# HarryL-Git/ampnet

Measured on AMD Instinct MI355X. Metric: AMPConv edges/sec (fwd+bwd), higher is better.
Workload: dtype f32

## Files before the change

### ampnet_amd/csrc/edge_mfma_bf16.hip

```cpp
#include "edge_wave16.h"

namespace {
using namespace wave16;

typedef unsigned short bf16_t;


#define MFMA_BF16(a, b, c) \
  __builtin_amdgcn_mfma_f32_16x16x32_bf16(__builtin_bit_cast(bf16x8, a), __builtin_bit_cast(bf16x8, b), (c), 0, 0, 0)

struct Args {
  ampconv_view_t Q, K, V, dO, O, dK, dV;
  const int32_t *ptr, *idx, *qidx;
  const float *cinv;
  HubArgs hub;
  int64_t n_units;
  int L, H;
  float qscale, oscale;
};

template <bool HALF>
__device__ __forceinline__ void store_tile(const ampconv_view_t &v, int64_t node, int h, const f32x4 (&T)[2][2],
                                           float scale, bool to_f32, int L, int lane) {
  const int g = lane >> 4;
#pragma unroll
  for (int nt = 0; nt < 2; ++nt) {
    const int i = (lane & 15) + 16 * nt;
    if (i < L) {
#pragma unroll
      for (int mc = 0; mc < (HALF ? 1 : 2); ++mc) {
        const float a = T[mc][nt][0] * scale, b = T[mc][nt][1] * scale, c = T[mc][nt][2] * scale,
                    d = T[mc][nt][3] * scale;
        const int64_t off = node * v.node_stride + (int64_t)h * v.head_stride + (int64_t)i * v.row_stride +
                            4 * g + 16 * mc;
        if (to_f32)
          *reinterpret_cast<float4 *>(reinterpret_cast<float *>(v.ptr) + off) = make_float4(a, b, c, d);
        else
          *reinterpret_cast<i32x2 *>(reinterpret_cast<bf16_t *>(v.ptr) + off) =
              i32x2{cvt_pk_bf16(a, b), cvt_pk_bf16(c, d)};
      }
    }
  }
}

struct FmtB {
  using Args = ::Args;
  static constexpr int kPlanes = 1, kElemBytes = 2, kLoOff = 0, kTileBytes = kPlaneBytes;
  using Frag = wave16::Frag<1>;
  template <bool HALF> using Geom = PairGeom<4, 3, HALF ? 2 : 4, 1>;
  static constexpr bool kHalfZeroLds = false;
  template <bool HALF> static constexpr int mc_tiles() { return 2; }
  static constexpr bool kShadow = false;
  static constexpr float kMasked = kNegBig, kPMul = 1.f;

  static __device__ __forceinline__ f32x4 mma(const Frag &a, const Frag &b, f32x4 c) { return MFMA_BF16(a.p[0], b.p[0], c); }
  static __device__ __forceinline__ Frag cd_frag(const f32x4 &t0, const f32x4 &t1) {
    return Frag{{i32x4{cvt_pk_bf16(t0[0], t0[1]), cvt_pk_bf16(t0[2], t0[3]), cvt_pk_bf16(t1[0], t1[1]),
                       cvt_pk_bf16(t1[2], t1[3])}}};
  }

  struct Scales {
    float sc;
  };
  template <bool HALF> static __device__ __forceinline__ Scales scales(const Args &a) { return Scales{a.qscale}; }
  static __device__ __forceinline__ int64_t qrow(const Args &a, int64_t r) { return a.qidx ? uniform_ld(a.qidx + r) : r; }
  static __device__ __forceinline__ float fwd_scale(const Scales &, float mean) { return mean; }
  static __device__ __forceinline__ float ds_mul(const Args &, int deg, const Frag (&)[2]) {
    return deg > 0 ? 1.f / (float)deg : 0.f;
  }
  template <bool HALF> static __device__ __forceinline__ float dq_scale(const Args &a, const Scales &, float, bool hubp) {
    return hubp ? 1.f : a.oscale;
  }

  template <bool HALF>
  static __device__ __forceinline__ float store(const ampconv_view_t &v, int64_t node, int h, const f32x4 (&T)[2][2],
                                                float scale, bool hubp, int L, int lane) {
    store_tile<HALF>(v, node, h, T, scale, hubp, L, lane);
    return 0.f;
  }
  template <bool HALF>
  static __device__ __forceinline__ void store_zero(const ampconv_view_t &v, int64_t node, int h, int L, int lane) {
    f32x4 Z[2][2];
#pragma unroll
    for (int mc = 0; mc < 2; ++mc) Z[mc][0] = Z[mc][1] = f32x4{0.f, 0.f, 0.f, 0.f};
    store_tile<HALF>(v, node, h, Z, 0.f, false, L, lane);
  }
  static __device__ __forceinline__ void record_absmax(const Args &, float) {}
};

template <bool FULL, bool HALF>
__global__ __launch_bounds__(64 * kWavesPerBlock) void fwd_bf16(Args a) { fwd_body<FmtB, FULL, HALF>(a); }
template <bool FULL, bool HALF>
__global__ __launch_bounds__(64 * kWavesPerBlock) void bwd_dst_bf16(Args a) { bwd_dst_body<FmtB, FULL, false, HALF>(a); }

constexpr int kTile32 = 32 * kRowBytes;

__device__ __forceinline__ i32x4 rowfrag_plain(const char *tile, int nt, int lane) {
  const int n = lane & 15, kg = lane >> 4;
  return *reinterpret_cast<const i32x4 *>(tile + plane_off(16 * nt + n, kg));
}
__device__ __forceinline__ i32x4 colfrag32(const char *tile, int blk, int lane) {
  const int q = (lane >> 2) & 3, pp = lane & 3, kg = lane >> 4;
  const int ch = 2 * blk + (pp >> 1), half = (pp & 1) << 3;
  return tr_frag(tile + plane_off(8 * kg + q, ch) + half, tile + plane_off(8 * kg + 4 + q, ch) + half);
}
__device__ __forceinline__ void file_column(char *img, int i, const f32x4 &t0, float t1_0, int g) {
  *reinterpret_cast<i32x2 *>(img + plane_off(i, g >> 1) + 8 * (g & 1)) = i32x2{cvt_pk_bf16(t0[0], t0[1]), cvt_pk_bf16(t0[2], t0[3])};
  *reinterpret_cast<unsigned short *>(img + plane_off(i, 2) + 2 * g) = (unsigned short)cvt_pk_bf16(t1_0, 0.f);
}

template <bool FULL, bool HALF>
__global__ __launch_bounds__(64 * kWavesPerBlock) void bwd_src_bf16_tr(Args a) {
  using G = FmtB::Geom<HALF>;
  __shared__ __attribute__((aligned(16))) char lds_all[kWavesPerBlock][4 * kTile32];
  for_unit<FmtB, HALF>(a, a.dK, &a.dV, [&](const Unit &u) __attribute__((always_inline)) {
    const int lane = u.lane, h = u.h, beg = u.beg, end = u.end;
    const int L = a.L, n = lane & 15, g = lane >> 4;
    char *Qt = lds_all[u.wave], *Gt = Qt + kTile32, *Pi = Gt + kTile32, *Si = Pi + kTile32;

    i32x4 kA[2], vA[2];
    {
      const char *kb = slot_ptr<2>(a.K, u.row, h), *vb = slot_ptr<2>(a.V, u.row, h);
      const unsigned krb = (unsigned)a.K.row_stride * 2u, vrb = (unsigned)a.V.row_stride * 2u;
#pragma unroll
      for (int mt = 0; mt < 2; ++mt) {
        kA[mt] = frag_global<1, HALF, true>(kb, krb, mt, L, lane).p[0];
        vA[mt] = frag_global<1, HALF, true>(vb, vrb, mt, L, lane).p[0];
      }
    }
    lds_zero(Qt, 4 * kTile32, lane);
    f32x4 dKT[2][2], dVT[2][2];
#pragma unroll
    for (int mc = 0; mc < 2; ++mc)
      dKT[mc][0] = dKT[mc][1] = dVT[mc][0] = dVT[mc][1] = f32x4{0.f, 0.f, 0.f, 0.f};

    Pair16<G::NLD> qg;
    float inv = 0.f, inv_next = 0.f;
    IdxWindow win;
    const unsigned qrb = (unsigned)a.Q.row_stride * 2u, grb = (unsigned)a.dO.row_stride * 2u;
    auto fetch = [&](int p, float &w) {
      const int64_t d = idxwin_get<true>(win, a.idx, a.cinv, p, end, lane, &w);
      pair16_load<FULL, G>(qg, slot_ptr<2>(a.Q, d, h), qrb, slot_ptr<2>(a.dO, d, h), grb, L, lane);
    };
    if (beg < end) {
      idxwin_load<true>(win, a.idx, a.cinv, beg, end, lane);
      fetch(beg, inv_next);
    }
    for (int p = beg; p < end; ++p) {
      pair16_to_lds<FULL, G, kTile32>(Qt, qg, L, lane);
      inv = inv_next;
      if (p + 1 < end) fetch(p + 1, inv_next);
      __builtin_amdgcn_wave_barrier();

      f32x4 S[2][2], dP[2][2];
#pragma unroll
      for (int nt = 0; nt < 2; ++nt) {
        const i32x4 qB = rowfrag_plain(Qt, nt, lane), gB = rowfrag_plain(Gt, nt, lane);
#pragma unroll
        for (int mt = 0; mt < 2; ++mt) {
          S[mt][nt] = MFMA_BF16(kA[mt], qB, (f32x4{0.f, 0.f, 0.f, 0.f}));
          dP[mt][nt] = MFMA_BF16(vA[mt], gB, (f32x4{0.f, 0.f, 0.f, 0.f}));
        }
      }
#pragma unroll
      for (int nt = 0; nt < 2; ++nt) {
        column_softmax<FULL>(S[0][nt], S[1][nt], a.qscale, 1.f, kNegBig, L, g);
        float part = S[1][nt][0] * dP[1][nt][0];
#pragma unroll
        for (int q = 0; q < 4; ++q) part = fmaf(S[0][nt][q], dP[0][nt][q], part);
        const float delta = groups_sum(part);
#pragma unroll
        for (int q = 0; q < 4; ++q) {
          dP[0][nt][q] = S[0][nt][q] * (dP[0][nt][q] - delta) * inv;
          S[0][nt][q] *= inv;
        }
        dP[1][nt][0] = S[1][nt][0] * (dP[1][nt][0] - delta) * inv;
        S[1][nt][0] *= inv;
        const int i = 16 * nt + n;
        if (i < kLmax && (FULL || i < L)) {
          file_column(Pi, i, S[0][nt], S[1][nt][0], g);
          file_column(Si, i, dP[0][nt], dP[1][nt][0], g);
        }
      }
      __builtin_amdgcn_wave_barrier();
      i32x4 pB[2], sB[2], gC[2], qC[2];
#pragma unroll
      for (int nt = 0; nt < 2; ++nt) {
        pB[nt] = colfrag32(Pi, nt, lane);
        sB[nt] = colfrag32(Si, nt, lane);
      }
#pragma unroll
      for (int mc = 0; mc < (HALF ? 1 : 2); ++mc) {
        gC[mc] = colfrag32(Gt, mc, lane);
        qC[mc] = colfrag32(Qt, mc, lane);
      }
      TR_FRAG_FENCE();
#pragma unroll
      for (int mc = 0; mc < (HALF ? 1 : 2); ++mc) {
        dVT[mc][0] = MFMA_BF16(gC[mc], pB[0], dVT[mc][0]);
        dVT[mc][1] = MFMA_BF16(gC[mc], pB[1], dVT[mc][1]);
        dKT[mc][0] = MFMA_BF16(qC[mc], sB[0], dKT[mc][0]);
        dKT[mc][1] = MFMA_BF16(qC[mc], sB[1], dKT[mc][1]);
      }
      __builtin_amdgcn_sched_barrier(0);
      asm volatile("s_nop 7" ::: "memory");
      __builtin_amdgcn_wave_barrier();
    }
    const bool hubp = a.hub.mode == 2;
    store_tile<HALF>(a.dK, u.onode, h, dKT, hubp ? 1.f : a.oscale, hubp, L, lane);
    store_tile<HALF>(a.dV, u.onode, h, dVT, 1.f, hubp, L, lane);
  });
}

typedef void (*EdgeKernel)(Args);
int launch(Args &a, int L, int D, int H, EdgeKernel const (&kernels)[2][2], hipStream_t stream) {
  const int dh = D / H;
  if (dh != DH && dh != DH / 2) return AMPCONV_E_BADARG;
  a.qscale = kLog2e / sqrtf((float)dh);
  a.oscale = 1.f / sqrtf((float)dh);
  return launch_wave16(kernels, a, L, dh == DH / 2, stream);
}

inline bool aligned16h(const ampconv_view_t &v) {
  return ((uintptr_t)v.ptr % 16 == 0) && (v.node_stride % 8 == 0) && (v.row_stride % 8 == 0) &&
         (v.head_stride % 8 == 0);
}

}

bool ampconv_bf16_supported(int L, int D, int H, const ampconv_view_t *views, int n) {
  if (!(L >= 1 && L <= kLmax && (D / H == DH || D / H == DH / 2) && D % H == 0)) return false;
  for (int i = 0; i < n; ++i)
    if (!aligned16h(views[i])) return false;
  return true;
}

int ampconv_fwd_edge_bf16(ampconv_view_t Q, ampconv_view_t K, ampconv_view_t V, const int32_t *rowptr,
                          const int32_t *col, const int32_t *qidx, int64_t n_rows, int L, int D, int H,
                          ampconv_view_t O, HubArgs hub, hipStream_t stream) {
  Args a{};
  a.Q = Q; a.K = K; a.V = V; a.O = O;
  a.ptr = rowptr; a.idx = col; a.qidx = qidx; a.hub = hub;
  a.n_units = n_rows * H; a.L = L; a.H = H;
  static const EdgeKernel kernels[2][2] = WAVE16_KERNELS(fwd_bf16);
  return launch(a, L, D, H, kernels, stream);
}

int ampconv_bwd_edge_dst_bf16(ampconv_view_t Q, ampconv_view_t K, ampconv_view_t V, ampconv_view_t dO,
                              const int32_t *rowptr, const int32_t *col, int64_t n_rows, int L, int D,
                              int H, ampconv_view_t dQ, HubArgs hub, hipStream_t stream) {
  Args a{};
  a.Q = Q; a.K = K; a.V = V; a.dO = dO; a.O = dQ;
  a.ptr = rowptr; a.idx = col; a.hub = hub;
  a.n_units = n_rows * H; a.L = L; a.H = H;
  static const EdgeKernel kernels[2][2] = WAVE16_KERNELS(bwd_dst_bf16);
  return launch(a, L, D, H, kernels, stream);
}

int ampconv_bwd_edge_src_bf16(ampconv_view_t Q, ampconv_view_t K, ampconv_view_t V, ampconv_view_t dO,
                              const int32_t *cscptr, const int32_t *crow, const float *cinv,
                              int64_t n_src, int L, int D, int H, ampconv_view_t dK, ampconv_view_t dV,
                              HubArgs hub, hipStream_t stream) {
  Args a{};
  a.Q = Q; a.K = K; a.V = V; a.dO = dO; a.dK = dK; a.dV = dV;
  a.ptr = cscptr; a.idx = crow; a.cinv = cinv; a.hub = hub;
  a.n_units = n_src * H; a.L = L; a.H = H;
  static const EdgeKernel kernels[2][2] = WAVE16_KERNELS(bwd_src_bf16_tr);
  return launch(a, L, D, H, kernels, stream);
}
```

### ampnet_amd/csrc/edge_mfma_f16x2.hip

```cpp
#include "edge_wave16.h"

namespace {
using namespace wave16;

constexpr int kLoOff = kPlaneBytes + 64;
constexpr int kTileBytes = kLoOff + kPlaneBytes;
constexpr float kPScale = 16384.f;
constexpr float kPUnscale = 1.f / 16384.f;
constexpr float kSqrtDh = 5.656854249492381f;
constexpr float kMasked = -__builtin_inff();

#define MFMA_F16(a, b, c) \
  __builtin_amdgcn_mfma_f32_16x16x32_f16(__builtin_bit_cast(f16x8, a), __builtin_bit_cast(f16x8, b), (c), 0, 0, 0)

__device__ __forceinline__ f32x4 mfma3(const i32x4 &ah, const i32x4 &al, const i32x4 &bh, const i32x4 &bl, f32x4 c) {
  c = MFMA_F16(al, bh, c);
  c = MFMA_F16(ah, bl, c);
  return MFMA_F16(ah, bh, c);
}

__device__ __forceinline__ float tile_max_norm2(const i32x4 &f0, const i32x4 &f1) {
  const float t = fmaxf(groups_sum(frag_sumsq(f0)), groups_sum(frag_sumsq(f1)));
  return __builtin_bit_cast(float, __builtin_amdgcn_readfirstlane(__builtin_bit_cast(int, row16_max(t))));
}
__device__ __forceinline__ float ds_scale(float own2, float other) {
  return plane_scale(2.f * __builtin_sqrtf(own2) * (kSqrtDh * other));
}

__device__ __forceinline__ void cd_frag2(const f32x4 &t0, float t1_0, i32x4 &hi, i32x4 &lo) {
  int h0, l0, h1, l1, h2, l2;
  split2(t0[0], t0[1], h0, l0);
  split2(t0[2], t0[3], h1, l1);
  split2(t1_0, 0.f, h2, l2);
  hi = i32x4{h0, h1, h2, 0};
  lo = i32x4{l0, l1, l2, 0};
}

struct Args {
  ampconv_view_t Q, K, V, dO, O, dK, dV;
  const int32_t *ptr, *idx;
  const float *bounds;
  float *absmax;
  const int32_t *spos;
  float *stats;
  HubArgs hub;
  int64_t n_units;
  int L, H;
};

template <bool QUARTER, int MC>
__device__ __forceinline__ float store_tile(const ampconv_view_t &v, int64_t node, int h, const f32x4 (&T)[MC][2],
                                            float scale, int L, int lane) {
  const int g = lane >> 4, n = lane & 15;
  float m = 0.f;
#pragma unroll
  for (int nt = 0; nt < 2; ++nt) {
    const int i = nt == 0 ? n : (QUARTER ? 16 + (n >> 2) : 16 + n);
    if (i < L && (nt == 0 || !QUARTER || (n & 3) == 0)) {
#pragma unroll
      for (int mc = 0; mc < MC; ++mc) {
        const float4 o = make_float4(T[mc][nt][0] * scale, T[mc][nt][1] * scale, T[mc][nt][2] * scale,
                                     T[mc][nt][3] * scale);
        const int64_t off = node * v.node_stride + (int64_t)h * v.head_stride + (int64_t)i * v.row_stride + 4 * g + 16 * mc;
        *reinterpret_cast<float4 *>(reinterpret_cast<float *>(v.ptr) + off) = o;
        m = finite_abs_max(m, o);
      }
    }
  }
  return m;
}

struct FmtP {
  using Args = ::Args;
  static constexpr int kPlanes = 2, kElemBytes = 4, kLoOff = ::kLoOff, kTileBytes = ::kTileBytes;
  using Frag = wave16::Frag<2>;
  template <bool HALF> using Geom = PairGeom<HALF ? 4 : 8, HALF ? 3 : 5, HALF ? 4 : 8, 2, ::kLoOff>;
  static constexpr bool kHalfZeroLds = true;
  template <bool HALF> static constexpr int mc_tiles() { return HALF ? 1 : 2; }
  static constexpr bool kShadow = true;
  static constexpr float kMasked = ::kMasked, kPMul = kPScale;

  static __device__ __forceinline__ f32x4 mma(const Frag &a, const Frag &b, f32x4 c) { return mfma3(a.p[0], a.p[1], b.p[0], b.p[1], c); }
  static __device__ __forceinline__ Frag cd_frag(const f32x4 &t0, const f32x4 &t1) {
    Frag f;
    cd_frag2(t0, t1[0], f.p[0], f.p[1]);
    return f;
  }

  struct Scales {
    float uq, ug, sc;
  };
  template <bool HALF> static constexpr float inv_sqrt_dh() { return HALF ? 0.25f : 0.17677669529663687f; }
  template <bool HALF> static __device__ __forceinline__ Scales scales(const Args &a) {
    const float uq = 1.f / plane_scale(uniform_ld(a.bounds)), ug = 1.f / plane_scale(uniform_ld(a.bounds + 1));
    return Scales{uq, ug, (kLog2e * inv_sqrt_dh<HALF>() * uq) * uq};
  }
  static __device__ __forceinline__ int64_t qrow(const Args &, int64_t r) { return r; }
  static __device__ __forceinline__ float fwd_scale(const Scales &k, float mean) { return kPUnscale * k.uq * mean; }
  static __device__ __forceinline__ float ds_mul(const Args &a, int, const Frag (&gB)[2]) {
    return ds_scale(tile_max_norm2(gB[0].p[0], gB[1].p[0]), uniform_ld(a.bounds + 2) * plane_scale(uniform_ld(a.bounds)));
  }
  template <bool HALF> static __device__ __forceinline__ float dq_scale(const Args &, const Scales &k, float ss, bool hubp) {
    return (((1.f / ss) * k.uq) * k.ug) * k.uq * (hubp ? 1.f : inv_sqrt_dh<HALF>());
  }

  template <bool HALF>
  static __device__ __forceinline__ float store(const ampconv_view_t &v, int64_t node, int h, const f32x4 (&T)[HALF ? 1 : 2][2],
                                                float scale, bool, int L, int lane) {
    return store_tile<false, HALF ? 1 : 2>(v, node, h, T, scale, L, lane);
  }
  template <bool HALF>
  static __device__ __forceinline__ void store_zero(const ampconv_view_t &v, int64_t node, int h, int L, int lane) {
    constexpr int MC = HALF ? 1 : 2;
    f32x4 Z[MC][2];
#pragma unroll
    for (int mc = 0; mc < MC; ++mc) Z[mc][0] = Z[mc][1] = f32x4{0.f, 0.f, 0.f, 0.f};
    store_tile<false, MC>(v, node, h, Z, 0.f, L, lane);
  }
  static __device__ __forceinline__ void record_absmax(const Args &a, float m) {
    if (a.absmax) wave_record_absmax(a.absmax, m);
  }
};

template <bool FULL, bool HALF>
__global__ __launch_bounds__(64 * kWavesPerBlock, 4) void fwd_f16x2(Args a) { fwd_body<FmtP, FULL, HALF>(a); }
template <bool FULL, bool STATS, bool HALF>
__global__ __launch_bounds__(64 * kWavesPerBlock, 3) void bwd_dst_f16x2(Args a) { bwd_dst_body<FmtP, FULL, STATS, HALF>(a); }

constexpr int kSrcLds = 4 * kTileBytes + 2 * kLmax * 4 + 32;
template <bool FULL, bool STATS, bool HALF>
__global__ __launch_bounds__(64 * kWavesPerBlock, 3) void bwd_src_f16x2(Args a) {
  using G = FmtP::Geom<HALF>;
  constexpr int MC = HALF ? 1 : 2;
  __shared__ __attribute__((aligned(16))) char lds_all[kWavesPerBlock][kSrcLds];
  for_unit<FmtP, HALF>(a, a.dK, &a.dV, [&](const Unit &u) __attribute__((always_inline)) {
    const int lane = u.lane, h = u.h, beg = u.beg, end = u.end;
    const int L = a.L, n = lane & 15;
    char *Qt = lds_all[u.wave], *Gt = Qt + kTileBytes, *Ko = Gt + kTileBytes, *Vo = Ko + kTileBytes;
    const FmtP::Scales k = FmtP::scales<HALF>(a);
    const float ug = k.ug, sc = k.sc;

    if (!FULL || HALF) lds_zero(Qt, 4 * kTileBytes, lane);
    Pair16<G::NLD> qg;
    pair16_load<FULL, G>(qg, slot_ptr<4>(a.K, u.row, h), (unsigned)a.K.row_stride * 4u, slot_ptr<4>(a.V, u.row, h),
                       (unsigned)a.V.row_stride * 4u, L, lane);
    pair16_to_lds<FULL, G, kTileBytes>(Ko, qg, L, lane);
    __builtin_amdgcn_wave_barrier();
    const float ss = ds_scale(tile_max_norm2(rowfrag(Vo, 0, lane), rowfrag(Vo, 1, lane)), uniform_ld(a.bounds + 3) * plane_scale(uniform_ld(a.bounds + 1)));
    f32x4 dKT[MC][2], dVT[MC][2];
#pragma unroll
    for (int mc = 0; mc < MC; ++mc)
      dKT[mc][0] = dKT[mc][1] = dVT[mc][0] = dVT[mc][1] = f32x4{0.f, 0.f, 0.f, 0.f};

    IdxWindow win;
    const unsigned qrb = (unsigned)a.Q.row_stride * 4u, grb = (unsigned)a.dO.row_stride * 4u;
    float *stl = reinterpret_cast<float *>(Vo + kTileBytes);
    float sv = 0.f;
    auto fetch = [&](int p) {
      const int64_t d = idxwin_get<false>(win, a.idx, nullptr, p, end, lane, nullptr);
      pair16_load<FULL, G>(qg, slot_ptr<4>(a.Q, d, h), qrb, slot_ptr<4>(a.dO, d, h), grb, L, lane);
      if (STATS && lane < kStatsPerUnit) sv = a.stats[((int64_t)p * a.H + h) * kStatsPerUnit + lane];
    };
    if (beg < end) {
      idxwin_load<false>(win, a.idx, nullptr, beg, end, lane);
      fetch(beg);
    }
    const bool v0 = FULL || n < L, v1 = (n & 3) == 0 && 16 + (n >> 2) < L;
    for (int p = beg; p < end; ++p) {
      pair16_to_lds<FULL, G, kTileBytes>(Qt, qg, L, lane);
      if (STATS && lane < kStatsPerUnit) stl[lane] = sv;
      if (p + 1 < end) fetch(p + 1);
      __builtin_amdgcn_wave_barrier();

      f32x4 S[2][2], dP[2][2];
      {
        i32x4 kh[2], kl[2], vh[2], vl[2];
#pragma unroll
        for (int nt = 0; nt < 2; ++nt) {
          kh[nt] = rowfrag(Ko, nt, lane);
          kl[nt] = rowfrag(Ko + kLoOff, nt, lane);
          vh[nt] = rowfrag(Vo, nt, lane);
          vl[nt] = rowfrag(Vo + kLoOff, nt, lane);
        }
#pragma unroll
        for (int mt = 0; mt < 2; ++mt) {
          const i32x4 ah = rowfrag(Qt, mt, lane), al = rowfrag(Qt + kLoOff, mt, lane);
          const i32x4 bh = rowfrag(Gt, mt, lane), bl = rowfrag(Gt + kLoOff, mt, lane);
#pragma unroll
          for (int nt = 0; nt < 2; ++nt) {
            S[mt][nt] = mfma3(ah, al, kh[nt], kl[nt], f32x4{0.f, 0.f, 0.f, 0.f});
            dP[mt][nt] = mfma3(bh, bl, vh[nt], vl[nt], f32x4{0.f, 0.f, 0.f, 0.f});
          }
        }
      }
      if (STATS) {
        const int g = lane >> 4;
        const f32x4 l0 = *reinterpret_cast<const f32x4 *>(stl + 4 * g), d0 = *reinterpret_cast<const f32x4 *>(stl + kLmax + 4 * g);
        const float l1 = stl[16 + g], d1 = stl[kLmax + 16 + g];
#pragma unroll
        for (int mt = 0; mt < 2; ++mt) {
#pragma unroll
          for (int q = 0; q < (mt == 0 ? 4 : 1); ++q) {
            const bool vr = FULL || (mt == 0 ? 4 * g + q : 16 + g) < L;
            const float ls = !vr ? 0.f : mt == 0 ? l0[q] : l1, dl = !vr ? 0.f : mt == 0 ? d0[q] : d1;
            const float s0 = (v0 && vr) ? S[mt][0][q] : kMasked, s1 = (v1 && vr) ? S[mt][1][q] : kMasked;
            const float p0 = fast_exp2(fmaf(s0, sc, -ls)), p1 = fast_exp2(fmaf(s1, sc, -ls));
            S[mt][0][q] = p0 * kPScale;
            S[mt][1][q] = p1 * kPScale;
            dP[mt][0][q] = p0 * (dP[mt][0][q] - dl) * ss;
            dP[mt][1][q] = p1 * (dP[mt][1][q] - dl) * ss;
          }
        }
      } else {
#pragma unroll
      for (int mt = 0; mt < 2; ++mt) {
#pragma unroll
        for (int q = 0; q < (mt == 0 ? 4 : 1); ++q) {
          const float s0 = v0 ? S[mt][0][q] : kMasked, s1 = v1 ? S[mt][1][q] : kMasked;
          const float m = row16_max(fmaxf(s0, s1));
          float p0 = fast_exp2((s0 - m) * sc), p1 = fast_exp2((s1 - m) * sc);
          const float rinv = fast_rcp(row16_sum(p0 + p1));
          p0 *= rinv;
          p1 *= rinv;
          const float delta = row16_sum(fmaf(p0, dP[mt][0][q], p1 * dP[mt][1][q]));
          S[mt][0][q] = p0 * kPScale;
          S[mt][1][q] = p1 * kPScale;
          dP[mt][0][q] = p0 * (dP[mt][0][q] - delta) * ss;
          dP[mt][1][q] = p1 * (dP[mt][1][q] - delta) * ss;
        }
      }
      }
      {
        i32x4 ph[2], pl[2], gh[MC], gl[MC];
        TR_PRE_READ();
#pragma unroll
        for (int mc = 0; mc < MC; ++mc) {
          gh[mc] = colfrag(Gt, mc, lane);
          gl[mc] = colfrag(Gt + kLoOff, mc, lane);
        }
#pragma unroll
        for (int nt = 0; nt < 2; ++nt) cd_frag2(S[0][nt], S[1][nt][0], ph[nt], pl[nt]);
        TR_FRAG_FENCE();
#pragma unroll
        for (int mc = 0; mc < MC; ++mc)
#pragma unroll
          for (int nt = 0; nt < 2; ++nt) dVT[mc][nt] = mfma3(gh[mc], gl[mc], ph[nt], pl[nt], dVT[mc][nt]);
        TR_WAR_GUARD();
      }
      {
        i32x4 sh[2], sl[2], qh[MC], ql[MC];
#pragma unroll
        for (int mc = 0; mc < MC; ++mc) {
          qh[mc] = colfrag(Qt, mc, lane);
          ql[mc] = colfrag(Qt + kLoOff, mc, lane);
        }
#pragma unroll
        for (int nt = 0; nt < 2; ++nt) cd_frag2(dP[0][nt], dP[1][nt][0], sh[nt], sl[nt]);
        TR_FRAG_FENCE();
#pragma unroll
        for (int mc = 0; mc < MC; ++mc)
#pragma unroll
          for (int nt = 0; nt < 2; ++nt) dKT[mc][nt] = mfma3(qh[mc], ql[mc], sh[nt], sl[nt], dKT[mc][nt]);
      }
      __builtin_amdgcn_wave_barrier();
    }
    const bool hubp = a.hub.mode == 2;
    float m = store_tile<true, MC>(a.dK, u.onode, h, dKT, FmtP::dq_scale<HALF>(a, k, ss, hubp), L, lane);
    m = fmaxf(m, store_tile<true, MC>(a.dV, u.onode, h, dVT, kPUnscale * ug, L, lane));
    FmtP::record_absmax(a, m);
  });
}

typedef void (*EdgeKernel)(Args);
int launch_fwd(Args &a, int L, bool half, hipStream_t st) {
  static const EdgeKernel k[2][2] = WAVE16_KERNELS(fwd_f16x2);
  return launch_wave16(k, a, L, half, st);
}
int launch_dst(Args &a, int L, bool half, hipStream_t st) {
  static const EdgeKernel k[2][2][2] = {WAVE16_KERNELS_STATS(bwd_dst_f16x2, false), WAVE16_KERNELS_STATS(bwd_dst_f16x2, true)};
  return launch_wave16(k[a.stats != nullptr], a, L, half, st);
}
int launch_src(Args &a, int L, bool half, hipStream_t st) {
  static const EdgeKernel k[2][2][2] = {WAVE16_KERNELS_STATS(bwd_src_f16x2, false), WAVE16_KERNELS_STATS(bwd_src_f16x2, true)};
  return launch_wave16(k[a.stats != nullptr], a, L, half, st);
}

inline bool plane_view_ok(const ampconv_view_t &v, int dh) {
  return v.ptr && ((uintptr_t)v.ptr % 16 == 0) && v.head_stride == dh && (v.node_stride % 4 == 0) && (v.row_stride % 4 == 0);
}
inline bool f32_view_ok(const ampconv_view_t &v) {
  return v.ptr && ((uintptr_t)v.ptr % 16 == 0) && (v.head_stride % 4 == 0) && (v.node_stride % 4 == 0) && (v.row_stride % 4 == 0);
}
int check_shape(int64_t n, int L, int D, int H, const float *bounds) {
  if (L <= 0 || D <= 0 || H <= 0 || D % H != 0 || n < 0 || !bounds) return AMPCONV_E_BADARG;
  if (L > kLmax || (D / H != DH && D / H != DH / 2)) return AMPCONV_E_DTYPE;
  return AMPCONV_OK;
}

}

extern "C" int ampconv_planes_supported(int L, int D, int H) {
  return L >= 1 && L <= kLmax && H > 0 && D % H == 0 && (D / H == DH || D / H == DH / 2);
}

extern "C" int ampconv_fwd_edge_planes(ampconv_view_t Q, ampconv_view_t K, ampconv_view_t V, const int32_t *rowptr,
                                       const int32_t *col, int64_t n_rows, int L, int D, int H, ampconv_view_t O,
                                       const void *hub_plan, int64_t hub_chunks, void *hub_ws, const float *bounds,
                                       void *stream) {
  if (int rc = check_shape(n_rows, L, D, H, bounds)) return rc;
  if (n_rows == 0) return AMPCONV_OK;
  if (!plane_view_ok(Q, D / H) || !plane_view_ok(K, D / H) || !plane_view_ok(V, D / H) || !f32_view_ok(O) || !rowptr) return AMPCONV_E_BADARG;
  hipStream_t st = (hipStream_t)stream;
  Args a{};
  a.Q = Q; a.K = K; a.V = V;
  a.ptr = rowptr; a.idx = col; a.bounds = bounds; a.L = L; a.H = H;
  auto run = [&](int64_t n, HubArgs hub, const ampconv_view_t *o, float *) {
    a.hub = hub; a.n_units = n * H; a.O = o[0];
    return launch_fwd(a, L, D / H == DH / 2, st);
  };
  return run_edge_pass(run, n_rows, {O}, hub_plan, hub_chunks, hub_ws, L, D, H, rowptr, {1.f}, 0, nullptr, st);
}

extern "C" int ampconv_bwd_edge_dst_planes(ampconv_view_t Q, ampconv_view_t K, ampconv_view_t V, ampconv_view_t dObar,
                                           const int32_t *rowptr, const int32_t *col, int64_t n_rows, int L, int D, int H,
                                           ampconv_view_t dQ, const void *hub_plan, int64_t hub_chunks, void *hub_ws,
                                           const float *bounds, const int32_t *spos, float *stats, float *out_absmax,
                                           void *stream) {
  if (int rc = check_shape(n_rows, L, D, H, bounds)) return rc;
  if (stats && (!spos || (uintptr_t)stats % 16 != 0)) return AMPCONV_E_BADARG;
  if (n_rows == 0) return AMPCONV_OK;
  if (!plane_view_ok(Q, D / H) || !plane_view_ok(K, D / H) || !plane_view_ok(V, D / H) || !plane_view_ok(dObar, D / H) || !f32_view_ok(dQ) || !rowptr)
    return AMPCONV_E_BADARG;
  hipStream_t st = (hipStream_t)stream;
  Args a{};
  a.Q = Q; a.K = K; a.V = V; a.dO = dObar;
  a.ptr = rowptr; a.idx = col; a.bounds = bounds; a.L = L; a.H = H;
  a.spos = spos; a.stats = stats;
  auto run = [&](int64_t n, HubArgs hub, const ampconv_view_t *o, float *absmax) {
    a.hub = hub; a.n_units = n * H; a.O = o[0]; a.absmax = absmax;
    return launch_dst(a, L, D / H == DH / 2, st);
  };
  return run_edge_pass(run, n_rows, {dQ}, hub_plan, hub_chunks, hub_ws, L, D, H, nullptr,
                       {1.f / sqrtf((float)(D / H))}, 0, out_absmax, st);
}

extern "C" int ampconv_bwd_edge_src_planes(ampconv_view_t Q, ampconv_view_t K, ampconv_view_t V, ampconv_view_t dObar,
                                           const int32_t *cscptr, const int32_t *crow, int64_t n_src, int L, int D, int H,
                                           ampconv_view_t dK, ampconv_view_t dV, const void *hub_plan, int64_t hub_chunks,
                                           void *hub_ws, const float *bounds, const float *stats, float *out_absmax,
                                           void *stream) {
  if (int rc = check_shape(n_src, L, D, H, bounds)) return rc;
  if (stats && (uintptr_t)stats % 16 != 0) return AMPCONV_E_BADARG;
  if (n_src == 0) return AMPCONV_OK;
  if (!plane_view_ok(Q, D / H) || !plane_view_ok(K, D / H) || !plane_view_ok(V, D / H) || !plane_view_ok(dObar, D / H) || !f32_view_ok(dK) ||
      !f32_view_ok(dV) || !cscptr)
    return AMPCONV_E_BADARG;
  hipStream_t st = (hipStream_t)stream;
  Args a{};
  a.Q = Q; a.K = K; a.V = V; a.dO = dObar;
  a.ptr = cscptr; a.idx = crow; a.bounds = bounds; a.L = L; a.H = H;
  a.stats = const_cast<float *>(stats);
  auto run = [&](int64_t n, HubArgs hub, const ampconv_view_t *o, float *absmax) {
    a.hub = hub; a.n_units = n * H; a.dK = o[0]; a.dV = o[1]; a.absmax = absmax;
    return launch_src(a, L, D / H == DH / 2, st);
  };
  return run_edge_pass(run, n_src, {dK, dV}, hub_plan, hub_chunks, hub_ws, L, D, H, nullptr,
                       {1.f / sqrtf((float)(D / H)), 1.f}, 0, out_absmax, st);
}
```

### ampnet_amd/csrc/edge_wave16.h

```cpp
#pragma once
#include "plane16.h"

namespace wave16 {
using namespace plane16;

constexpr int kWavesPerBlock = 4;
constexpr int DH = 32;
constexpr int kRowBytes = DH * 2;
constexpr int kPlaneBytes = kLmax * kRowBytes;

template <int P>
struct Frag {
  i32x4 p[P];
};

struct Unit {
  int lane, wave;
  int64_t row, onode;
  int h, beg, end, deg;
};
template <class Fmt, bool HALF, class Body>
__device__ __forceinline__ void for_unit(const typename Fmt::Args &a, const ampconv_view_t &out0, const ampconv_view_t *out1,
                                         const Body &body) {
  Unit u;
  u.lane = threadIdx.x & 63;
  u.wave = __builtin_amdgcn_readfirstlane(threadIdx.x >> 6);
  const int64_t unit = (int64_t)blockIdx.x * kWavesPerBlock + u.wave;
  if (unit >= a.n_units) return;
  if (!map_unit(a.hub, a.ptr, unit, a.n_units, a.H, u.row, u.onode, u.h, u.beg, u.end, u.deg)) return;
  if (u.beg >= u.end && a.hub.mode != 2) {
    Fmt::template store_zero<HALF>(out0, u.onode, u.h, a.L, u.lane);
    if (out1) Fmt::template store_zero<HALF>(*out1, u.onode, u.h, a.L, u.lane);
    return;
  }
  body(u);
}

template <class T>
__device__ __forceinline__ T uniform_ld(const T *p) {
  return *(const __attribute__((address_space(4))) T *)p;
}

template <int EB>
__device__ __forceinline__ const char *slot_ptr(const ampconv_view_t &v, int64_t n, int h) {
  return reinterpret_cast<const char *>(v.ptr) + EB * (n * v.node_stride + (int64_t)h * v.head_stride);
}

template <int LPR_, int NLD_, int CHUNKS_, int PLANES_, int LO_OFF_ = 0>
struct PairGeom {
  static constexpr int LPR = LPR_, RPL = 64 / LPR_, NLD = NLD_, CHUNKS = CHUNKS_, CPP = LPR_ / PLANES_, LO_OFF = LO_OFF_;
};
template <int N>
struct Pair16 {
  i32x4 v[N];
};

template <bool FULL, class G>
__device__ __forceinline__ void pair16_load(Pair16<G::NLD> &t, const char *baseA, unsigned strideA, const char *baseB,
                                          unsigned strideB, int L, int lane) {
  const int r = lane / G::LPR, q = lane % G::LPR;
#pragma unroll
  for (int i = 0; i < G::NLD; ++i) {
    const int R = r + G::RPL * i;
    const bool isB = R >= kLmax;
    const int j = isB ? R - kLmax : R;
    const bool valid = (R < 2 * kLmax) && (FULL || j < L) && (G::CHUNKS == G::LPR || q < G::CHUNKS);
    if (G::CHUNKS < G::LPR) t.v[i] = i32x4{0, 0, 0, 0};
    const unsigned off = (unsigned)j * (isB ? strideB : strideA) + 16u * (unsigned)q;
    const char *p = (isB ? baseB : baseA) + off;
    if (valid) t.v[i] = *reinterpret_cast<const i32x4 *>(p);
  }
}

template <bool FULL, class G, int TILE>
__device__ __forceinline__ void pair16_to_lds(char *tileA, const Pair16<G::NLD> &t, int L, int lane) {
  const int r = lane / G::LPR, q = lane % G::LPR;
#pragma unroll
  for (int i = 0; i < G::NLD; ++i) {
    const int R = r + G::RPL * i;
    const bool isB = R >= kLmax;
    const int j = isB ? R - kLmax : R;
    if ((R < 2 * kLmax) && (FULL || j < L))
      *reinterpret_cast<i32x4 *>(tileA + (isB ? TILE : 0) + (G::CPP < G::LPR && q >= G::CPP ? G::LO_OFF : 0) +
                                 plane_off(j, G::CPP < G::LPR ? q % G::CPP : q)) = t.v[i];
  }
}

__device__ __forceinline__ void lds_zero(char *p, int bytes, int lane) {
  int *z = reinterpret_cast<int *>(p);
  for (int i = lane; i < bytes / 4; i += AMPCONV_WAVE) z[i] = 0;
}

template <int P, bool HALF, bool QUARTER>
__device__ __forceinline__ Frag<P> frag_global(const char *base, unsigned row_bytes, int t, int L, int lane) {
  const int m = lane & 15, kg = lane >> 4;
  const int j = t == 0 ? m : 16 + (QUARTER ? m >> 2 : m);
  Frag<P> f;
#pragma unroll
  for (int pl = 0; pl < P; ++pl) f.p[pl] = i32x4{0, 0, 0, 0};
  if (j < L && (!HALF || kg < 2)) {
#pragma unroll
    for (int pl = P - 1; pl >= 0; --pl)
      f.p[pl] = *reinterpret_cast<const i32x4 *>(base + (unsigned)j * row_bytes + pl * (HALF ? kRowBytes / 2 : kRowBytes) + 16 * kg);
  }
  return f;
}
template <class Fmt>
__device__ __forceinline__ typename Fmt::Frag lds_rowfrag(const char *img, int mt, int lane) {
  typename Fmt::Frag f;
#pragma unroll
  for (int pl = 0; pl < Fmt::kPlanes; ++pl) f.p[pl] = rowfrag(img + pl * Fmt::kLoOff, mt, lane);
  return f;
}
template <class Fmt>
__device__ __forceinline__ typename Fmt::Frag lds_colfrag(const char *img, int mc, int lane) {
  typename Fmt::Frag f;
#pragma unroll
  for (int pl = 0; pl < Fmt::kPlanes; ++pl) f.p[pl] = colfrag(img + pl * Fmt::kLoOff, mc, lane);
  return f;
}

template <bool FULL>
__device__ __forceinline__ float column_softmax(f32x4 &t0, f32x4 &t1, float sc, float mul, float masked, int L, int g) {
  if (!FULL) {
#pragma unroll
    for (int q = 0; q < 4; ++q)
      if (4 * g + q >= L) t0[q] = masked;
    if (16 + g >= L) t1[0] = masked;
  }
  float m = fmaxf(fmaxf(fmaxf(t0[0], t0[1]), fmaxf(t0[2], t0[3])), t1[0]);
  m = groups_max(m);
#pragma unroll
  for (int q = 0; q < 4; ++q) t0[q] = fast_exp2((t0[q] - m) * sc);
  t1[0] = fast_exp2((t1[0] - m) * sc);
  float l = ((t0[0] + t0[1]) + (t0[2] + t0[3])) + t1[0];
  l = groups_sum(l);
  const float inv = fast_rcp(l) * mul;
#pragma unroll
  for (int q = 0; q < 4; ++q) t0[q] *= inv;
  t1[0] *= inv;
  t1[1] = t1[2] = t1[3] = 0.f;
  return fmaf(m, sc, __builtin_amdgcn_logf(l));
}

template <class Fmt, bool FULL, bool HALF>
__device__ __forceinline__ void fwd_body(const typename Fmt::Args &a) {
  using F = typename Fmt::Frag;
  using G = typename Fmt::template Geom<HALF>;
  constexpr int MC = Fmt::template mc_tiles<HALF>(), TB = Fmt::kTileBytes, EB = Fmt::kElemBytes;
  __shared__ __attribute__((aligned(16))) char lds_all[kWavesPerBlock][2 * TB];
  for_unit<Fmt, HALF>(a, a.O, nullptr, [&](const Unit &u) __attribute__((always_inline)) {
    const int lane = u.lane, h = u.h, beg = u.beg, end = u.end;
    const int L = a.L, g = lane >> 4;
    char *Kt = lds_all[u.wave], *Vt = Kt + TB;
    const typename Fmt::Scales k = Fmt::template scales<HALF>(a);

    F qB[2];
    {
      const char *qb = slot_ptr<EB>(a.Q, Fmt::qrow(a, u.row), h);
      const unsigned rb = (unsigned)a.Q.row_stride * EB;
#pragma unroll
      for (int nt = 0; nt < 2; ++nt) qB[nt] = frag_global<Fmt::kPlanes, HALF, false>(qb, rb, nt, L, lane);
    }
    if (!FULL || (HALF && Fmt::kHalfZeroLds)) lds_zero(Kt, 2 * TB, lane);
    f32x4 OT[MC][2];
#pragma unroll
    for (int mc = 0; mc < MC; ++mc) OT[mc][0] = OT[mc][1] = f32x4{0.f, 0.f, 0.f, 0.f};

    Pair16<G::NLD> kv;
    IdxWindow win;
    const unsigned krb = (unsigned)a.K.row_stride * EB, vrb = (unsigned)a.V.row_stride * EB;
    auto fetch = [&](int p) {
      const int64_t s = idxwin_get<false>(win, a.idx, nullptr, p, end, lane, nullptr);
      pair16_load<FULL, G>(kv, slot_ptr<EB>(a.K, s, h), krb, slot_ptr<EB>(a.V, s, h), vrb, L, lane);
    };
    if (beg < end) {
      idxwin_load<false>(win, a.idx, nullptr, beg, end, lane);
      fetch(beg);
    }
    for (int p = beg; p < end; ++p) {
      pair16_to_lds<FULL, G, TB>(Kt, kv, L, lane);
      if (p + 1 < end) fetch(p + 1);
      __builtin_amdgcn_wave_barrier();

      f32x4 S[2][2];
#pragma unroll
      for (int mt = 0; mt < 2; ++mt) {
        const F kA = lds_rowfrag<Fmt>(Kt, mt, lane);
#pragma unroll
        for (int nt = 0; nt < 2; ++nt) S[mt][nt] = Fmt::mma(kA, qB[nt], f32x4{0.f, 0.f, 0.f, 0.f});
      }
      F pB[2];
#pragma unroll
      for (int nt = 0; nt < 2; ++nt) {
        column_softmax<FULL>(S[0][nt], S[1][nt], k.sc, Fmt::kPMul, Fmt::kMasked, L, g);
        if (!Fmt::kShadow) pB[nt] = Fmt::cd_frag(S[0][nt], S[1][nt]);
      }
      F vA[MC];
      if (Fmt::kShadow) TR_PRE_READ();
#pragma unroll
      for (int mc = 0; mc < MC; ++mc) vA[mc] = lds_colfrag<Fmt>(Vt, mc, lane);
      if (Fmt::kShadow) {
#pragma unroll
        for (int nt = 0; nt < 2; ++nt) pB[nt] = Fmt::cd_frag(S[0][nt], S[1][nt]);
      }
      TR_FRAG_FENCE();
#pragma unroll
      for (int mc = 0; mc < MC; ++mc)
#pragma unroll
        for (int nt = 0; nt < 2; ++nt) OT[mc][nt] = Fmt::mma(vA[mc], pB[nt], OT[mc][nt]);
      __builtin_amdgcn_wave_barrier();
    }
    const bool hubp = a.hub.mode == 2;
    Fmt::template store<HALF>(a.O, u.onode, h, OT, Fmt::fwd_scale(k, hubp ? 1.f : (u.deg > 0 ? 1.f / (float)u.deg : 0.f)),
                              hubp, L, lane);
  });
}

template <class Fmt, bool FULL, bool STATS, bool HALF>
__device__ __forceinline__ void bwd_dst_body(const typename Fmt::Args &a) {
  using F = typename Fmt::Frag;
  using G = typename Fmt::template Geom<HALF>;
  constexpr int MC = Fmt::template mc_tiles<HALF>(), TB = Fmt::kTileBytes, EB = Fmt::kElemBytes;
  __shared__ __attribute__((aligned(16))) char lds_all[kWavesPerBlock][2 * TB];
  for_unit<Fmt, HALF>(a, a.O, nullptr, [&](const Unit &u) __attribute__((always_inline)) {
    const int lane = u.lane, h = u.h, beg = u.beg, end = u.end;
    const int L = a.L, g = lane >> 4;
    char *Kt = lds_all[u.wave], *Vt = Kt + TB;
    const typename Fmt::Scales k = Fmt::template scales<HALF>(a);

    F qB[2], gB[2];
    {
      const char *qb = slot_ptr<EB>(a.Q, u.row, h), *gb = slot_ptr<EB>(a.dO, u.row, h);
      const unsigned qrb = (unsigned)a.Q.row_stride * EB, grb = (unsigned)a.dO.row_stride * EB;
#pragma unroll
      for (int nt = 0; nt < 2; ++nt) {
        qB[nt] = frag_global<Fmt::kPlanes, HALF, false>(qb, qrb, nt, L, lane);
        gB[nt] = frag_global<Fmt::kPlanes, HALF, false>(gb, grb, nt, L, lane);
      }
    }
    const float dsm = Fmt::ds_mul(a, u.deg, gB);
    if (!FULL || (HALF && Fmt::kHalfZeroLds)) lds_zero(Kt, 2 * TB, lane);
    f32x4 dQT[MC][2];
#pragma unroll
    for (int mc = 0; mc < MC; ++mc) dQT[mc][0] = dQT[mc][1] = f32x4{0.f, 0.f, 0.f, 0.f};

    Pair16<G::NLD> kv;
    IdxWindow win;
    const unsigned krb = (unsigned)a.K.row_stride * EB, vrb = (unsigned)a.V.row_stride * EB;
    const float *sposf = nullptr;
    if constexpr (STATS) sposf = reinterpret_cast<const float *>(a.spos);
    float cposf = 0.f, cposf_next = 0.f;
    auto fetch = [&](int p) {
      const int64_t s = idxwin_get<STATS>(win, a.idx, sposf, p, end, lane, &cposf_next);
      pair16_load<FULL, G>(kv, slot_ptr<EB>(a.K, s, h), krb, slot_ptr<EB>(a.V, s, h), vrb, L, lane);
    };
    if (beg < end) {
      idxwin_load<STATS>(win, a.idx, sposf, beg, end, lane);
      fetch(beg);
    }
    for (int p = beg; p < end; ++p) {
      pair16_to_lds<FULL, G, TB>(Kt, kv, L, lane);
      cposf = cposf_next;
      if (p + 1 < end) fetch(p + 1);
      __builtin_amdgcn_wave_barrier();

      f32x4 S[2][2], dP[2][2];
      float lse[2], dlt[2];
#pragma unroll
      for (int mt = 0; mt < 2; ++mt) {
        const F kA = lds_rowfrag<Fmt>(Kt, mt, lane);
        const F vA = lds_rowfrag<Fmt>(Vt, mt, lane);
#pragma unroll
        for (int nt = 0; nt < 2; ++nt) {
          S[mt][nt] = Fmt::mma(kA, qB[nt], f32x4{0.f, 0.f, 0.f, 0.f});
          dP[mt][nt] = Fmt::mma(vA, gB[nt], f32x4{0.f, 0.f, 0.f, 0.f});
        }
      }
      F sB[2];
#pragma unroll
      for (int nt = 0; nt < 2; ++nt) {
        lse[nt] = column_softmax<FULL>(S[0][nt], S[1][nt], k.sc, 1.f, Fmt::kMasked, L, g);
        float part = S[1][nt][0] * dP[1][nt][0];
#pragma unroll
        for (int q = 0; q < 4; ++q) part = fmaf(S[0][nt][q], dP[0][nt][q], part);
        const float delta = groups_sum(part);
        dlt[nt] = delta;
#pragma unroll
        for (int q = 0; q < 4; ++q) S[0][nt][q] *= (dP[0][nt][q] - delta) * dsm;
        S[1][nt][0] *= (dP[1][nt][0] - delta) * dsm;
        if (!Fmt::kShadow) sB[nt] = Fmt::cd_frag(S[0][nt], S[1][nt]);
      }
      F kC[MC];
      if (Fmt::kShadow) TR_PRE_READ();
#pragma unroll
      for (int mc = 0; mc < MC; ++mc) kC[mc] = lds_colfrag<Fmt>(Kt, mc, lane);
      if (Fmt::kShadow) {
#pragma unroll
        for (int nt = 0; nt < 2; ++nt) sB[nt] = Fmt::cd_frag(S[0][nt], S[1][nt]);
      }
      TR_FRAG_FENCE();
#pragma unroll
      for (int mc = 0; mc < MC; ++mc)
#pragma unroll
        for (int nt = 0; nt < 2; ++nt) dQT[mc][nt] = Fmt::mma(kC[mc], sB[nt], dQT[mc][nt]);
      if constexpr (STATS) {
        float *st = a.stats + ((int64_t)__builtin_bit_cast(int, cposf) * a.H + h) * kStatsPerUnit;
        if (lane < L) {
          st[lane] = lane < 16 ? lse[0] : lse[1];
          st[kLmax + lane] = lane < 16 ? dlt[0] : dlt[1];
        }
      }
      __builtin_amdgcn_wave_barrier();
    }
    const bool hubp = a.hub.mode == 2;
    const float m = Fmt::template store<HALF>(a.O, u.onode, h, dQT, Fmt::template dq_scale<HALF>(a, k, dsm, hubp), hubp, L, lane);
    Fmt::record_absmax(a, m);
  });
}

#define WAVE16_KERNELS(K) {{K<false, false>, K<true, false>}, {K<false, true>, K<true, true>}}
#define WAVE16_KERNELS_STATS(K, S) {{K<false, S, false>, K<true, S, false>}, {K<false, S, true>, K<true, S, true>}}
template <class Args>
int launch_wave16(void (*const (&kernels)[2][2])(Args), const Args &a, int L, bool half, hipStream_t stream) {
  return launch_wave_units(kernels[half][L == kLmax], a, kWavesPerBlock, stream);
}

}
```

### ampnet_amd/csrc/plane16.h

```cpp
#pragma once
#include "mfma_tile.h"

namespace plane16 {

typedef int i32x4 __attribute__((ext_vector_type(4)));
typedef int i32x2 __attribute__((ext_vector_type(2)));
typedef float f32x2 __attribute__((ext_vector_type(2)));
typedef short s16x4 __attribute__((ext_vector_type(4)));
typedef _Float16 f16x2 __attribute__((ext_vector_type(2)));
typedef _Float16 f16x8 __attribute__((ext_vector_type(8)));
typedef __bf16 bf16x2 __attribute__((ext_vector_type(2)));
typedef __bf16 bf16x8 __attribute__((ext_vector_type(8)));

constexpr float kLog2e = 1.4426950408889634f;

__device__ __forceinline__ int cvt_pk_bf16(float a, float b) {
  f32x2 v = {a, b};
  return __builtin_bit_cast(int, __builtin_convertvector(v, bf16x2));
}
__device__ __forceinline__ int cvt_pk_f16(float a, float b) {
  f32x2 v = {a, b};
  return __builtin_bit_cast(int, __builtin_convertvector(v, f16x2));
}

__device__ __forceinline__ float plane_scale(float bound) {
  int e = (int)((__builtin_bit_cast(unsigned, bound) >> 23) & 0xFFu);
  e = e < 15 ? 15 : (e > 254 ? 254 : e);
  return __builtin_bit_cast(float, (unsigned)(268 - e) << 23);
}
__device__ __forceinline__ float plane_unscale(float bound) { return 1.f / plane_scale(bound); }

__device__ __forceinline__ void split2(float x0, float x1, int &h, int &l) {
  h = cvt_pk_f16(x0, x1);
  const f16x2 hv = __builtin_bit_cast(f16x2, h);
  l = cvt_pk_f16(x0 - (float)hv[0], x1 - (float)hv[1]);
}

__device__ __forceinline__ float frag_sumsq(const i32x4 &f) {
  float s = 0.f;
#pragma unroll
  for (int k = 0; k < 4; ++k) {
    const f16x2 v = __builtin_bit_cast(f16x2, f[k]);
    s = __builtin_amdgcn_fdot2(v, v, s, false);
  }
  return s;
}

__device__ __forceinline__ i32x2 tr_half(const char *p) {
  return __builtin_bit_cast(i32x2, __builtin_amdgcn_ds_read_tr16_b64_v4i16((__attribute__((address_space(3))) s16x4 *)p));
}
__device__ __forceinline__ i32x4 tr_frag(const char *p0, const char *p1) {
  const i32x2 ai = tr_half(p0), bi = tr_half(p1);
  return i32x4{ai[0], ai[1], bi[0], bi[1]};
}

#define TR_FRAG_FENCE()                                    \
  do {                                                     \
    __builtin_amdgcn_sched_barrier(0);                     \
    asm volatile("s_waitcnt lgkmcnt(0)" ::: "memory");     \
    __builtin_amdgcn_sched_barrier(0);                     \
  } while (0)
#define TR_FRAG_FENCE_IDLE()                                                          \
  do {                                                                                \
    __builtin_amdgcn_sched_barrier(0);                                                \
    asm volatile("s_waitcnt lgkmcnt(0)\n\ts_nop 7\n\ts_nop 7" ::: "memory");          \
    __builtin_amdgcn_sched_barrier(0);                                                \
  } while (0)
#define TR_WAR_GUARD()                         \
  do {                                         \
    __builtin_amdgcn_sched_barrier(0);         \
    asm volatile("s_nop 7" ::: "memory");      \
    __builtin_amdgcn_sched_barrier(0);         \
  } while (0)
#define TR_PRE_READ() asm volatile("s_nop 7" ::: "memory")

constexpr int kPlaneRowBytes = 64;
__device__ __forceinline__ int plane_off(int j, int ch) {
  const int f = (4 - (j >> 2)) & 3;
  return j * kPlaneRowBytes + ((ch ^ f) << 4);
}
__device__ __forceinline__ i32x4 rowfrag(const char *img, int mt, int lane) {
  const int m = lane & 15, kg = lane >> 4;
  const int j = mt == 0 ? m : 16 + (m >> 2);
  return *reinterpret_cast<const i32x4 *>(img + plane_off(j, kg));
}
__device__ __forceinline__ i32x4 colfrag(const char *img, int mc, int lane) {
  const int q = (lane >> 2) & 3, pp = lane & 3, kg = lane >> 4;
  const int ch = 2 * mc + (pp >> 1), half = (pp & 1) << 3;
  return tr_frag(img + plane_off(4 * kg + q, ch) + half, img + plane_off(16 + kg, ch) + half);
}

}
```

Measured before the change: 26.43 million.

## Pack split-f16 operands so the three-MFMA compensated product uses two MFMAs

Replaces the three-MFMA hi/lo split-precision product in the f16x2 path with a packed operand layout, where the K dimension carries hi and lo terms (and the short tail row) so that two MFMAs compute the same compensated sum. Column fragments are read with a third transpose read that selects hi or lo plane per lane, and the B fragments are built as duplicated hi/lo pairs. The aim is to cut matrix-core instruction count in the P·V, dV, dK and dQ products, in exchange for a more intricate fragment construction and reliance on unused K padding slots.

Measured after the change: 26.33 million. Within noise of the previous version (-0.4%).

```diff
diff --git a/ampnet_amd/csrc/edge_mfma_bf16.hip b/ampnet_amd/csrc/edge_mfma_bf16.hip
--- a/ampnet_amd/csrc/edge_mfma_bf16.hip
+++ b/ampnet_amd/csrc/edge_mfma_bf16.hip
@@ -54,7 +54,11 @@
   static constexpr float kMasked = kNegBig, kPMul = 1.f;
 
   static __device__ __forceinline__ f32x4 mma(const Frag &a, const Frag &b, f32x4 c) { return MFMA_BF16(a.p[0], b.p[0], c); }
-  static __device__ __forceinline__ Frag cd_frag(const f32x4 &t0, const f32x4 &t1) {
+  using TokA = Frag;
+  using TokB = Frag;
+  static __device__ __forceinline__ Frag tok_a(const char *img, int mc, int lane) { return Frag{{colfrag(img, mc, lane)}}; }
+  static __device__ __forceinline__ f32x4 tok_mma(const Frag &a, const Frag &b, f32x4 c) { return mma(a, b, c); }
+  static __device__ __forceinline__ Frag tok_b(const f32x4 &t0, const f32x4 &t1) {
     return Frag{{i32x4{cvt_pk_bf16(t0[0], t0[1]), cvt_pk_bf16(t0[2], t0[3]), cvt_pk_bf16(t1[0], t1[1]),
                        cvt_pk_bf16(t1[2], t1[3])}}};
   }
diff --git a/ampnet_amd/csrc/edge_mfma_f16x2.hip b/ampnet_amd/csrc/edge_mfma_f16x2.hip
--- a/ampnet_amd/csrc/edge_mfma_f16x2.hip
+++ b/ampnet_amd/csrc/edge_mfma_f16x2.hip
@@ -27,13 +27,9 @@
   return plane_scale(2.f * __builtin_sqrtf(own2) * (kSqrtDh * other));
 }
 
-__device__ __forceinline__ void cd_frag2(const f32x4 &t0, float t1_0, i32x4 &hi, i32x4 &lo) {
-  int h0, l0, h1, l1, h2, l2;
-  split2(t0[0], t0[1], h0, l0);
-  split2(t0[2], t0[3], h1, l1);
-  split2(t1_0, 0.f, h2, l2);
-  hi = i32x4{h0, h1, h2, 0};
-  lo = i32x4{l0, l1, l2, 0};
+__device__ __forceinline__ f32x4 mfma_packed(const PackedA &a, const PackedB &b, f32x4 c) {
+  c = MFMA_F16(a.m2, b.m2, c);
+  return MFMA_F16(a.m1, b.m1, c);
 }
 
 struct Args {
@@ -81,11 +77,11 @@
   static constexpr float kMasked = ::kMasked, kPMul = kPScale;
 
   static __device__ __forceinline__ f32x4 mma(const Frag &a, const Frag &b, f32x4 c) { return mfma3(a.p[0], a.p[1], b.p[0], b.p[1], c); }
-  static __device__ __forceinline__ Frag cd_frag(const f32x4 &t0, const f32x4 &t1) {
-    Frag f;
-    cd_frag2(t0, t1[0], f.p[0], f.p[1]);
-    return f;
-  }
+  using TokA = PackedA;
+  using TokB = PackedB;
+  static __device__ __forceinline__ PackedA tok_a(const char *img, int mc, int lane) { return colfrag_packed(img, ::kLoOff, mc, lane); }
+  static __device__ __forceinline__ PackedB tok_b(const f32x4 &t0, const f32x4 &t1) { return cd_frag_packed(t0, t1[0]); }
+  static __device__ __forceinline__ f32x4 tok_mma(const PackedA &a, const PackedB &b, f32x4 c) { return mfma_packed(a, b, c); }
 
   struct Scales {
     float uq, ug, sc;
@@ -231,36 +227,32 @@
       }
       }
       {
-        i32x4 ph[2], pl[2], gh[MC], gl[MC];
+        PackedA gA[MC];
+        PackedB pB[2];
         TR_PRE_READ();
 #pragma unroll
-        for (int mc = 0; mc < MC; ++mc) {
-          gh[mc] = colfrag(Gt, mc, lane);
-          gl[mc] = colfrag(Gt + kLoOff, mc, lane);
-        }
-#pragma unroll
-        for (int nt = 0; nt < 2; ++nt) cd_frag2(S[0][nt], S[1][nt][0], ph[nt], pl[nt]);
+        for (int mc = 0; mc < MC; ++mc) gA[mc] = FmtP::tok_a(Gt, mc, lane);
+#pragma unroll
+        for (int nt = 0; nt < 2; ++nt) pB[nt] = FmtP::tok_b(S[0][nt], S[1][nt]);
         TR_FRAG_FENCE();
 #pragma unroll
         for (int mc = 0; mc < MC; ++mc)
 #pragma unroll
-          for (int nt = 0; nt < 2; ++nt) dVT[mc][nt] = mfma3(gh[mc], gl[mc], ph[nt], pl[nt], dVT[mc][nt]);
+          for (int nt = 0; nt < 2; ++nt) dVT[mc][nt] = FmtP::tok_mma(gA[mc], pB[nt], dVT[mc][nt]);
         TR_WAR_GUARD();
       }
       {
-        i32x4 sh[2], sl[2], qh[MC], ql[MC];
-#pragma unroll
-        for (int mc = 0; mc < MC; ++mc) {
-          qh[mc] = colfrag(Qt, mc, lane);
-          ql[mc] = colfrag(Qt + kLoOff, mc, lane);
-        }
-#pragma unroll
-        for (int nt = 0; nt < 2; ++nt) cd_frag2(dP[0][nt], dP[1][nt][0], sh[nt], sl[nt]);
+        PackedA qA[MC];
+        PackedB sB[2];
+#pragma unroll
+        for (int mc = 0; mc < MC; ++mc) qA[mc] = FmtP::tok_a(Qt, mc, lane);
+#pragma unroll
+        for (int nt = 0; nt < 2; ++nt) sB[nt] = FmtP::tok_b(dP[0][nt], dP[1][nt]);
         TR_FRAG_FENCE();
 #pragma unroll
         for (int mc = 0; mc < MC; ++mc)
 #pragma unroll
-          for (int nt = 0; nt < 2; ++nt) dKT[mc][nt] = mfma3(qh[mc], ql[mc], sh[nt], sl[nt], dKT[mc][nt]);
+          for (int nt = 0; nt < 2; ++nt) dKT[mc][nt] = FmtP::tok_mma(qA[mc], sB[nt], dKT[mc][nt]);
       }
       __builtin_amdgcn_wave_barrier();
     }
diff --git a/ampnet_amd/csrc/edge_wave16.h b/ampnet_amd/csrc/edge_wave16.h
--- a/ampnet_amd/csrc/edge_wave16.h
+++ b/ampnet_amd/csrc/edge_wave16.h
@@ -112,13 +112,6 @@
   for (int pl = 0; pl < Fmt::kPlanes; ++pl) f.p[pl] = rowfrag(img + pl * Fmt::kLoOff, mt, lane);
   return f;
 }
-template <class Fmt>
-__device__ __forceinline__ typename Fmt::Frag lds_colfrag(const char *img, int mc, int lane) {
-  typename Fmt::Frag f;
-#pragma unroll
-  for (int pl = 0; pl < Fmt::kPlanes; ++pl) f.p[pl] = colfrag(img + pl * Fmt::kLoOff, mc, lane);
-  return f;
-}
 
 template <bool FULL>
 __device__ __forceinline__ float column_softmax(f32x4 &t0, f32x4 &t1, float sc, float mul, float masked, int L, int g) {
@@ -190,25 +183,25 @@
 #pragma unroll
         for (int nt = 0; nt < 2; ++nt) S[mt][nt] = Fmt::mma(kA, qB[nt], f32x4{0.f, 0.f, 0.f, 0.f});
       }
-      F pB[2];
+      typename Fmt::TokB pB[2];
 #pragma unroll
       for (int nt = 0; nt < 2; ++nt) {
         column_softmax<FULL>(S[0][nt], S[1][nt], k.sc, Fmt::kPMul, Fmt::kMasked, L, g);
-        if (!Fmt::kShadow) pB[nt] = Fmt::cd_frag(S[0][nt], S[1][nt]);
-      }
-      F vA[MC];
+        if (!Fmt::kShadow) pB[nt] = Fmt::tok_b(S[0][nt], S[1][nt]);
+      }
+      typename Fmt::TokA vA[MC];
       if (Fmt::kShadow) TR_PRE_READ();
 #pragma unroll
-      for (int mc = 0; mc < MC; ++mc) vA[mc] = lds_colfrag<Fmt>(Vt, mc, lane);
+      for (int mc = 0; mc < MC; ++mc) vA[mc] = Fmt::tok_a(Vt, mc, lane);
       if (Fmt::kShadow) {
 #pragma unroll
-        for (int nt = 0; nt < 2; ++nt) pB[nt] = Fmt::cd_frag(S[0][nt], S[1][nt]);
+        for (int nt = 0; nt < 2; ++nt) pB[nt] = Fmt::tok_b(S[0][nt], S[1][nt]);
       }
       TR_FRAG_FENCE();
 #pragma unroll
       for (int mc = 0; mc < MC; ++mc)
 #pragma unroll
-        for (int nt = 0; nt < 2; ++nt) OT[mc][nt] = Fmt::mma(vA[mc], pB[nt], OT[mc][nt]);
+        for (int nt = 0; nt < 2; ++nt) OT[mc][nt] = Fmt::tok_mma(vA[mc], pB[nt], OT[mc][nt]);
       __builtin_amdgcn_wave_barrier();
     }
     const bool hubp = a.hub.mode == 2;
@@ -277,7 +270,7 @@
           dP[mt][nt] = Fmt::mma(vA, gB[nt], f32x4{0.f, 0.f, 0.f, 0.f});
         }
       }
-      F sB[2];
+      typename Fmt::TokB sB[2];
 #pragma unroll
       for (int nt = 0; nt < 2; ++nt) {
         lse[nt] = column_softmax<FULL>(S[0][nt], S[1][nt], k.sc, 1.f, Fmt::kMasked, L, g);
@@ -289,21 +282,21 @@
 #pragma unroll
         for (int q = 0; q < 4; ++q) S[0][nt][q] *= (dP[0][nt][q] - delta) * dsm;
         S[1][nt][0] *= (dP[1][nt][0] - delta) * dsm;
-        if (!Fmt::kShadow) sB[nt] = Fmt::cd_frag(S[0][nt], S[1][nt]);
-      }
-      F kC[MC];
+        if (!Fmt::kShadow) sB[nt] = Fmt::tok_b(S[0][nt], S[1][nt]);
+      }
+      typename Fmt::TokA kC[MC];
       if (Fmt::kShadow) TR_PRE_READ();
 #pragma unroll
-      for (int mc = 0; mc < MC; ++mc) kC[mc] = lds_colfrag<Fmt>(Kt, mc, lane);
+      for (int mc = 0; mc < MC; ++mc) kC[mc] = Fmt::tok_a(Kt, mc, lane);
       if (Fmt::kShadow) {
 #pragma unroll
-        for (int nt = 0; nt < 2; ++nt) sB[nt] = Fmt::cd_frag(S[0][nt], S[1][nt]);
+        for (int nt = 0; nt < 2; ++nt) sB[nt] = Fmt::tok_b(S[0][nt], S[1][nt]);
       }
       TR_FRAG_FENCE();
 #pragma unroll
       for (int mc = 0; mc < MC; ++mc)
 #pragma unroll
-        for (int nt = 0; nt < 2; ++nt) dQT[mc][nt] = Fmt::mma(kC[mc], sB[nt], dQT[mc][nt]);
+        for (int nt = 0; nt < 2; ++nt) dQT[mc][nt] = Fmt::tok_mma(kC[mc], sB[nt], dQT[mc][nt]);
       if constexpr (STATS) {
         float *st = a.stats + ((int64_t)__builtin_bit_cast(int, cposf) * a.H + h) * kStatsPerUnit;
         if (lane < L) {
diff --git a/ampnet_amd/csrc/plane16.h b/ampnet_amd/csrc/plane16.h
--- a/ampnet_amd/csrc/plane16.h
+++ b/ampnet_amd/csrc/plane16.h
@@ -90,4 +90,26 @@
   return tr_frag(img + plane_off(4 * kg + q, ch) + half, img + plane_off(16 + kg, ch) + half);
 }
 
+struct PackedA {
+  i32x4 m1, m2;
+};
+__device__ __forceinline__ PackedA colfrag_packed(const char *img, int lo_off, int mc, int lane) {
+  const int q = (lane >> 2) & 3, pp = lane & 3, kg = lane >> 4;
+  const int ch = 2 * mc + (pp >> 1), half = (pp & 1) << 3;
+  const int main_off = plane_off(4 * kg + q, ch) + half;
+  const i32x2 hm = tr_half(img + main_off), lm = tr_half(img + lo_off + main_off);
+  const i32x2 tm = tr_half(img + ((q & 1) ? lo_off : 0) + plane_off(16 + kg, ch) + half);
+  return PackedA{i32x4{hm[0], hm[1], lm[0], lm[1]}, i32x4{hm[0], hm[1], tm[0], tm[1]}};
 }
+struct PackedB {
+  i32x4 m1, m2;
+};
+__device__ __forceinline__ PackedB cd_frag_packed(const f32x4 &t0, float t1_0) {
+  int h0, l0, h1, l1, h2, l2;
+  split2(t0[0], t0[1], h0, l0);
+  split2(t0[2], t0[3], h1, l1);
+  split2(t1_0, t1_0, h2, l2);
+  return PackedB{i32x4{h0, h1, h0, h1}, i32x4{l0, l1, h2, l2}};
+}
+
+}
```
